# lauraflu/gr-doa

Measured on AMD Instinct MI355X. Metric: DoA snapshots/sec (autocorr+MUSIC+peak) @ N=4, 1024 samp, 1024 angles, higher is better.
Workload: dtype f32; 1 GPU; BASELINE.json configs[1]: 4-ch ULA, 1 source, K=1024 (overlap 0), P=1024, batch=4096 snapshots/step, complex fp32, SNR 20 dB; batch=4096, inputs=4, snapshot_size=1024, pspectrum_len=1024, num_targets=1, internal_precision=64, rotating_batches=8, hip_streams=4, parallelism=snapshot-sharded x1, no data-path collective

## Files before the change

### gr-doa_amd/csrc/autocorrelate.hip

```cpp
#include "common.hpp"

#include <cstdlib>

namespace doa {

struct CovArgs {
    const float2 *in[DOA_MAX_ANT_ELE];
    float2 *out;
    int n_ch;
    int K;
    int S;
    int n_out;
    int avg;
    float inv_k;
    float fb_hk;
    const float2 *gain;
    float2 *pieces;
    int q, r;
    int n_steps;
};

template <int TN> struct TriAcc {
    float d[TN];
    float re[TN * (TN - 1) / 2 > 0 ? TN * (TN - 1) / 2 : 1];
    float im[TN * (TN - 1) / 2 > 0 ? TN * (TN - 1) / 2 : 1];
};

template <int TN> __device__ __forceinline__ void tri_accumulate(TriAcc<TN> &acc, const float2 (&x)[TN])
{
    int idx = 0;
#pragma unroll
    for (int a = 0; a < TN; a++) {
        acc.d[a] = fmaf(x[a].x, x[a].x, fmaf(x[a].y, x[a].y, acc.d[a]));
#pragma unroll
        for (int b = a + 1; b < TN; b++) {
            acc.re[idx] = fmaf(x[a].x, x[b].x, fmaf(x[a].y, x[b].y, acc.re[idx]));
            acc.im[idx] = fmaf(x[a].y, x[b].x, fmaf(-x[a].x, x[b].y, acc.im[idx]));
            idx++;
        }
    }
}

template <int TN, bool VEC2, int UN, bool NT = false>
__global__ __launch_bounds__(256) void cov_wave_kernel(CovArgs g)
{
    const int lane = threadIdx.x & (kWave - 1);
    const int wave0 = blockIdx.x * (blockDim.x / kWave) + (threadIdx.x / kWave);
    const int n_waves = gridDim.x * (blockDim.x / kWave);
    for (int snap = wave0; snap < g.n_out; snap += n_waves) {
    const size_t base = (size_t)snap * (size_t)g.S;

    TriAcc<TN> acc;
#pragma unroll
    for (int a = 0; a < TN; a++) acc.d[a] = 0.f;
#pragma unroll
    for (int i = 0; i < TN * (TN - 1) / 2; i++) { acc.re[i] = 0.f; acc.im[i] = 0.f; }

    if constexpr (VEC2) {
        const int npair = g.K >> 1;
        int p = lane;
        for (; p + (UN - 1) * kWave < npair; p += UN * kWave) {
            float4 v[UN][TN];
#pragma unroll
            for (int u = 0; u < UN; u++)
#pragma unroll
                for (int a = 0; a < TN; a++)
                    v[u][a] = load_f4<NT>(reinterpret_cast<const float4 *>(g.in[a] + base + 2 * (size_t)(p + u * kWave)));
#pragma unroll
            for (int u = 0; u < UN; u++) {
                float2 x0[TN], x1[TN];
#pragma unroll
                for (int a = 0; a < TN; a++) { x0[a] = make_float2(v[u][a].x, v[u][a].y); x1[a] = make_float2(v[u][a].z, v[u][a].w); }
                tri_accumulate<TN>(acc, x0);
                tri_accumulate<TN>(acc, x1);
            }
        }
        for (; p < npair; p += kWave) {
            float4 v[TN];
#pragma unroll
            for (int a = 0; a < TN; a++) v[a] = load_f4<NT>(reinterpret_cast<const float4 *>(g.in[a] + base + 2 * (size_t)p));
            float2 x0[TN], x1[TN];
#pragma unroll
            for (int a = 0; a < TN; a++) { x0[a] = make_float2(v[a].x, v[a].y); x1[a] = make_float2(v[a].z, v[a].w); }
            tri_accumulate<TN>(acc, x0);
            tri_accumulate<TN>(acc, x1);
        }
        if ((g.K & 1) && lane == 0) {
            float2 x[TN];
#pragma unroll
            for (int a = 0; a < TN; a++) x[a] = g.in[a][base + (size_t)(g.K - 1)];
            tri_accumulate<TN>(acc, x);
        }
    } else {
#pragma unroll 4
        for (int t = lane; t < g.K; t += kWave) {
            float2 x[TN];
#pragma unroll
            for (int a = 0; a < TN; a++) x[a] = g.in[a][base + (size_t)t];
            tri_accumulate<TN>(acc, x);
        }
    }

#pragma unroll
    for (int a = 0; a < TN; a++) acc.d[a] = wave_allreduce_sum(acc.d[a]);
#pragma unroll
    for (int i = 0; i < TN * (TN - 1) / 2; i++) {
        acc.re[i] = wave_allreduce_sum(acc.re[i]);
        acc.im[i] = wave_allreduce_sum(acc.im[i]);
    }

    float2 r = make_float2(0.f, 0.f);
    {
        int idx = 0;
#pragma unroll
        for (int a = 0; a < TN; a++) {
            if (lane == a + a * TN) r = make_float2(acc.d[a], 0.f);
#pragma unroll
            for (int b = a + 1; b < TN; b++) {
                if (lane == a + b * TN) r = make_float2(acc.re[idx], acc.im[idx]);
                if (lane == b + a * TN) r = make_float2(acc.re[idx], -acc.im[idx]);
                idx++;
            }
        }
    }
    r.x = __fmul_rn(r.x, g.inv_k);
    r.y = __fmul_rn(r.y, g.inv_k);
    if (g.gain && lane < TN * TN) {
        const float2 w = g.gain[lane];
        r = make_float2(fmaf(w.x, r.x, -w.y * r.y), fmaf(w.x, r.y, w.y * r.x));
    }
    if (g.avg == 1) {
        const int src = (lane < TN * TN) ? (TN * TN - 1 - lane) : lane;
        const float px = __shfl(r.x, src, kWave);
        const float py = __shfl(r.y, src, kWave);
        r.x = __fadd_rn(__fmul_rn(0.5f, r.x), __fmul_rn(g.fb_hk, px));
        r.y = __fadd_rn(__fmul_rn(0.5f, r.y), __fmul_rn(g.fb_hk, -py));
    }
    if (lane < TN * TN) g.out[(size_t)snap * (TN * TN) + lane] = r;
    }
// ... 18 lines not shown
            for (int a = 0; a < TN; a++) { x0[a] = make_float2(v[u][a].x, v[u][a].y); x1[a] = make_float2(v[u][a].z, v[u][a].w); }
            tri_accumulate<TN>(acc, x0);
            tri_accumulate<TN>(acc, x1);
        }
    }
    for (; p < npair; p += kWave) {
        float4 v[TN];
#pragma unroll
        for (int a = 0; a < TN; a++) v[a] = load_f4<NT>(reinterpret_cast<const float4 *>(in[a] + first + 2 * (size_t)p));
        float2 x0[TN], x1[TN];
#pragma unroll
        for (int a = 0; a < TN; a++) { x0[a] = make_float2(v[a].x, v[a].y); x1[a] = make_float2(v[a].z, v[a].w); }
        tri_accumulate<TN>(acc, x0);
        tri_accumulate<TN>(acc, x1);
    }
}

template <int TN> __device__ __forceinline__ void tri_clear(TriAcc<TN> &acc)
{
#pragma unroll
    for (int a = 0; a < TN; a++) acc.d[a] = 0.f;
#pragma unroll
    for (int i = 0; i < TN * (TN - 1) / 2; i++) { acc.re[i] = 0.f; acc.im[i] = 0.f; }
}

template <int TN> __device__ __forceinline__ float2 tri_reduce_to_lane(TriAcc<TN> &acc, int lane)
{
#pragma unroll
    for (int a = 0; a < TN; a++) acc.d[a] = wave_allreduce_sum(acc.d[a]);
#pragma unroll
    for (int i = 0; i < TN * (TN - 1) / 2; i++) {
        acc.re[i] = wave_allreduce_sum(acc.re[i]);
        acc.im[i] = wave_allreduce_sum(acc.im[i]);
    }
    float2 r = make_float2(0.f, 0.f);
    int idx = 0;
#pragma unroll
    for (int a = 0; a < TN; a++) {
// ... 383 lines not shown
```

### gr-doa_amd/csrc/kernels.hpp

```cpp
#pragma once
#include "common.hpp"

namespace doa {

size_t autocorrelate_workspace_bytes(int N, int K, int ovl, int n_out);
int launch_autocorrelate(int N, int K, int ovl, int avg, int n_out, const void *const *d_in, void *d_out,
                         hipStream_t st, const void *d_gain_outer = nullptr, void *d_workspace = nullptr);

struct MusicTables {
    int N = 0, M = 0, P = 0;
    float norm_spacing = 0.f;
    DevBuf d_z;
    DevBuf d_zd;
    int build(float norm_spacing, int num_targets, int num_ant_ele, int pspectrum_len);
    void release() { d_z.release(); d_zd.release(); }
};

inline int coef_stride(int N) { return 2 * N; }

int launch_music_evd(int N, int M, int n_items, const void *d_R, void *d_coef, void *d_coef_d, void *d_pn,
                     int evd_bits, hipStream_t st, void *d_cheb = nullptr);
inline bool music_uses_cheb(int N, int bits) { return N <= 4 && bits == 64; }
constexpr int kChebRecord = 8;
long long evd_fallback_count(bool reset);
// ... 4 lines not shown
int launch_music_scan(const MusicTables &t, int bits, int n_items, const void *d_coef, void *d_spec, void *d_q,
                      hipStream_t st, const PeakTables *peaks = nullptr, void *d_max = nullptr,
                      void *d_argmax = nullptr, bool *peaks_done = nullptr, bool store_spectrum = true,
                      const void *d_cheb = nullptr);

struct PeakTables {
    int M = 0, L = 0;
    float x_min = 0.f, x_max = 0.f;
    DevBuf d_x;
    int build(int num_max_vals, int vector_len, float x_min, float x_max);
    void release() { d_x.release(); }
};
int launch_find_local_max(const PeakTables &t, int n_items, const void *d_in, void *d_max, void *d_argmax,
                          hipStream_t st);

int launch_root_music(int N, int M, float norm_spacing, int n_items, const void *d_coef, void *d_out,
                      void *d_status, hipStream_t st, void *d_roots = nullptr);
int launch_root_select(int N, int M, float norm_spacing, int n_items, const void *d_roots, void *d_out, void *d_status,
                       hipStream_t st);

}
```

### gr-doa_amd/csrc/music_evd.hip

```cpp
#include "jacobi.hpp"
#include "kernels.hpp"
#include <mutex>
#include <type_traits>

#include <cstdlib>

namespace doa {

}
#include "evd_subspace.hpp"
namespace doa {

__device__ __forceinline__ void write_cheb_record(double *__restrict__ o, const double (&ux)[4], const double (&uy)[4])
{
    o[0] = ux[0] - 2 * ux[2]; o[1] = 2 * ux[1] - 6 * ux[3]; o[2] = 4 * ux[2]; o[3] = 8 * ux[3];
    o[4] = 2 * uy[3] - 2 * uy[1]; o[5] = -4 * uy[2]; o[6] = -8 * uy[3]; o[7] = 0.0;
}

template <int N, typename T>
__global__ __launch_bounds__(64) void music_evd_kernel(const float2 *__restrict__ R, float *__restrict__ coef,
                                                       double *__restrict__ coef_d, float2 *__restrict__ pn_out,
                                                       int n_items, int M, double *__restrict__ cheb_d,
                                                       unsigned long long *__restrict__ fallback_count)
{
    const int item = blockIdx.x * blockDim.x + threadIdx.x;
    if (item >= n_items) return;
    T u[2 * N];
    const float2 *Ri = R + (size_t)item * (N * N);
    float2 *pn_i = pn_out ? pn_out + (size_t)item * (N * N) : nullptr;
    bool done = false;
    if constexpr (sizeof(T) == 8) {
        if (M == 1) {
            done = evd_small_subspace<N, 1>(Ri, u, pn_i);
            if (!done && fallback_count) atomicAdd(fallback_count, 1ull);
        }
    }
    if (!done) evd_item_coefficients<N, T>(Ri, M, u, pn_i);
    if (coef) {
#pragma unroll
        for (int k = 0; k < 2 * N; k++) coef[(size_t)item * (2 * N) + k] = (float)u[k];
    }
    if (coef_d) {
#pragma unroll
        for (int k = 0; k < 2 * N; k++) coef_d[(size_t)item * (2 * N) + k] = (double)u[k];
    }
    if (cheb_d) {
        const double ux[4] = {(double)u[0], (N > 1) ? (double)u[1] : 0.0, (N > 2) ? (double)u[3] : 0.0, (N > 3) ? (double)u[5] : 0.0};
        const double uy[4] = {0.0, (N > 1) ? (double)u[2] : 0.0, (N > 2) ? (double)u[4] : 0.0, (N > 3) ? (double)u[6] : 0.0};
        write_cheb_record(cheb_d + (size_t)item * kChebRecord, ux, uy);
    }
}

template <int G> struct Tournament {
    static constexpr int a(int t, int j) { return j == 0 ? G - 1 : (t + j) % (G - 1); }
    static constexpr int b(int t, int j) { return j == 0 ? t : (t - j + (G - 1)) % (G - 1); }
    static constexpr int p(int t, int j) { return a(t, j) < b(t, j) ? a(t, j) : b(t, j); }
    static constexpr int q(int t, int j) { return a(t, j) < b(t, j) ? b(t, j) : a(t, j); }
};

template <typename T> __device__ __forceinline__ T lane_fetch(T v, int src_lane);
template <> __device__ __forceinline__ float lane_fetch<float>(float v, int src_lane) { return __shfl(v, src_lane, kWave); }
template <> __device__ __forceinline__ double lane_fetch<double>(double v, int src_lane) { return __shfl(v, src_lane, kWave); }

template <int G, typename T> __device__ __forceinline__ T group_sum(T v, int lane)
{
// ... 967 lines not shown
```

### gr-doa_amd/csrc/pipeline.hip

```cpp
#include "kernels.hpp"
#include "pipeline_lanes.hpp"

#include <cstdlib>
#include <cstring>
#include <string>

namespace doa {
bool find_local_max_fast_ok(int L, const void *d_in);
int launch_find_local_max_serial(const PeakTables &t, int n_items, const void *d_in, void *d_max, void *d_argmax,
                                 void *d_scratch, hipStream_t st);
}

struct doa_music_pipeline {
    int N = 0, K = 0, ovl = 0, avg = 0;
    int max_batch = 0;
    int bits = 64;
    int device = 0;
    unsigned stages = 7;
    doa::MusicTables music;
    doa::PeakTables peaks;
    doa::DevBuf d_cov, d_coef, d_cheb, d_spec, d_scratch, d_gain;
    bool has_gain = false;
    hipStream_t hst[2] = {nullptr, nullptr};
    doa::DevBuf d_in[2], d_res;
    doa::DevBuf d_work[2];
    doa::PinnedBuf h_stage;
    int fail_chunk = -1;
    enum { kCoef = 0, kCheb, kCov, kSpec, kWork, kScratch };
    doa::PipeLanes lanes;
};

struct PipeWs {
    void *coef;
    void *cheb;
    void *spec_scratch;
    void *work;
    doa::DevBuf *scratch;
    size_t scratch_item_off;
};

static int run_k1(doa_music_pipeline *h, int n, const void *const *d_in, void *cov, const PipeWs &ws, hipStream_t st)
{
    if (~h->stages & 1u) return DOA_OK;
    return doa::launch_autocorrelate(h->N, h->K, h->ovl, h->avg, n, d_in, cov, st, h->has_gain ? h->d_gain.p : nullptr, ws.work);
// ... 33 lines not shown

static int run_dev(doa_music_pipeline *h, int n, const void *const *d_in, void *cov, void *spec, void *mx, void *am,
                   size_t item_off, hipStream_t st, int lane = 0)
{
    const bool dbl = (h->bits == 64);
    PipeWs ws;
    ws.coef = static_cast<char *>(h->d_coef.p) + item_off * doa::coef_stride(h->N) * (dbl ? sizeof(double) : sizeof(float));
    ws.cheb = h->d_cheb.p ? static_cast<char *>(h->d_cheb.p) + item_off * doa::kChebRecord * sizeof(double) : nullptr;
    ws.spec_scratch = static_cast<char *>(h->d_spec.p) + item_off * h->peaks.L * sizeof(float);
    ws.work = h->d_work[lane].p;
    ws.scratch = &h->d_scratch;
    ws.scratch_item_off = item_off;
    return run_ws(h, n, d_in, cov, spec, mx, am, ws, st);
}

extern "C" {

doa_music_pipeline_t *doa_music_pipeline_create(int inputs, int snapshot_size, int overlap_size, int avg_method,
                                                float norm_spacing, int num_targets, int pspectrum_len, int max_batch)
{
    doa::clear_error();
    if (inputs <= 0 || inputs > DOA_MAX_ANT_ELE || snapshot_size <= 0 || overlap_size < 0 ||
        overlap_size >= snapshot_size) {
        doa::set_error("music_pipeline: bad autocorrelate parameters (inputs=%d snapshot=%d overlap=%d)", inputs,
                       snapshot_size, overlap_size);
        return nullptr;
    }
    if (num_targets <= 0 || num_targets >= inputs || num_targets > DOA_MAX_PEAKS || !(norm_spacing > 0.0f) ||
        norm_spacing > 0.5f || pspectrum_len <= 0 || max_batch <= 0) {
        doa::set_error("music_pipeline: bad MUSIC parameters (norm_spacing=%g num_targets=%d inputs=%d "
// ... 17 lines not shown
    if (const size_t ws = doa::autocorrelate_workspace_bytes(inputs, snapshot_size, overlap_size, max_batch); ws && rc == DOA_OK)
        rc = h->d_work[0].reserve(ws);
    if (rc != DOA_OK) {
        doa_music_pipeline_destroy(h);
        return nullptr;
    }
    return h;
}

void doa_music_pipeline_destroy(doa_music_pipeline_t *h)
{
    if (!h) return;
    h->music.release();
    h->peaks.release();
    h->d_cov.release(); h->d_coef.release(); h->d_cheb.release(); h->d_spec.release(); h->d_scratch.release(); h->d_gain.release();
    h->d_res.release(); h->h_stage.release();
    for (auto &b : h->d_work) b.release();
    for (auto &b : h->d_in) b.release();
    for (auto st : h->hst)
        if (st) (void)hipStreamDestroy(st);
    h->lanes.release();
    delete h;
}

int doa_music_pipeline_fuse_antenna_correction(doa_music_pipeline_t *h, const float *gains_re_im)
{
    doa::clear_error();
    if (!h) return DOA_ERR_INVALID_ARG;
    if (!gains_re_im) { h->has_gain = false; return DOA_OK; }
    const int N = h->N;
    float2 w[DOA_MAX_ANT_ELE * DOA_MAX_ANT_ELE];
// ... 20 lines not shown
int doa_music_pipeline_work_dev(doa_music_pipeline_t *h, int noutput_items, const void *const *d_input_items,
                                void *d_cov_out, void *d_spectrum_out, void *d_max_out, void *d_argmax_out,
                                void *hip_stream)
{
    doa::clear_error();
    if (!h || noutput_items < 0 || !d_input_items || (noutput_items > 0 && (!d_max_out || !d_argmax_out))) {
        doa::set_error("music_pipeline_work_dev: bad arguments");
        return DOA_ERR_INVALID_ARG;
    }
    if (noutput_items > h->max_batch) {
        doa::set_error("music_pipeline_work_dev: noutput_items=%d exceeds max_batch=%d", noutput_items, h->max_batch);
        return DOA_ERR_INVALID_ARG;
    }
    if (noutput_items == 0) return 0;
    if (int brc = doa::bind_device(h->device); brc != DOA_OK) return brc;
    void *cov = d_cov_out ? d_cov_out : h->d_cov.p;
    void *spec = d_spectrum_out;
    return run_dev(h, noutput_items, d_input_items, cov, spec, d_max_out, d_argmax_out, 0,
                   static_cast<hipStream_t>(hip_stream));
}

int doa_music_pipeline_set_lanes(doa_music_pipeline_t *h, int n_lanes)
{
    doa::clear_error();
    if (!h || h->lanes.set_count(n_lanes) != DOA_OK) {
        doa::set_error("music_pipeline_set_lanes: need 1 <= n_lanes <= %d", doa::PipeLanes::kMaxLanes);
        return DOA_ERR_INVALID_ARG;
    }
    return DOA_OK;
}

int doa_music_pipeline_work_dev_batches(doa_music_pipeline_t *h, int n_batches, int noutput_items,
                                        const void *const *d_input_items, void *const *d_cov_out,
                                        void *const *d_spectrum_out, void *const *d_max_out, void *const *d_argmax_out,
// ... 6 lines not shown
    }
    if (noutput_items > h->max_batch) {
        doa::set_error("music_pipeline_work_dev_batches: noutput_items=%d exceeds max_batch=%d", noutput_items, h->max_batch);
        return DOA_ERR_INVALID_ARG;
    }
    for (int b = 0; b < n_batches; b++)
        if (noutput_items > 0 && (!d_max_out[b] || !d_argmax_out[b])) {
            doa::set_error("music_pipeline_work_dev_batches: batch %d has no peak output pointers", b);
            return DOA_ERR_INVALID_ARG;
        }
    if (n_batches == 0 || noutput_items == 0) return 0;
    if (int brc = doa::bind_device(h->device); brc != DOA_OK) return brc;
    const int N = h->N;
    const int fail_at = h->lanes.fail_batch;
    h->fail_chunk = -1;
    if (h->lanes.n_lanes == 1 && hip_stream != DOA_STREAM_DETACHED) {
        hipStream_t caller = static_cast<hipStream_t>(hip_stream);
        h->lanes.fail_batch = -1;
        for (int b = 0; b < n_batches; b++) {
            if (fail_at == b) {
                doa::set_error("music_pipeline_work_dev_batches: injected failure in batch %d", b);
                (void)hipStreamSynchronize(caller);
                return DOA_ERR_HIP;
            }
            void *cov = (d_cov_out && d_cov_out[b]) ? d_cov_out[b] : h->d_cov.p;
            const int rc = run_dev(h, noutput_items, d_input_items + (size_t)b * N, cov, d_spectrum_out ? d_spectrum_out[b] : nullptr,
                                   d_max_out[b], d_argmax_out[b], 0, caller);
            if (rc < 0) { (void)hipStreamSynchronize(caller); return rc; }
        }
        return n_batches * noutput_items;
// ... 200 lines not shown
```

### gr-doa_amd/csrc/pipeline_lanes.hpp

```cpp
#pragma once
#include "common.hpp"

#include <string>

namespace doa {

int create_lane_streams(const hipStream_t *have, int n_have, hipStream_t *out, int n_new);

inline int ensure_stream_pair(hipStream_t (&st)[2])
{
    for (int i = 0; i < 2; i++) {
        if (st[i]) continue;
        if (const int rc = create_lane_streams(&st[1 - i], st[1 - i] ? 1 : 0, &st[i], 1); rc != DOA_OK) return rc;
    }
    return DOA_OK;
}

struct PipeLane {
    hipStream_t st = nullptr;
    bool own_stream = true;
    hipEvent_t done = nullptr;
    static constexpr int kBufs = 6;
    DevBuf buf[kBufs];
};

struct PipeLanes {
    static constexpr int kMaxLanes = 8;
    PipeLane lanes[kMaxLanes];
    int n_lanes = 4;
    int next_lane = 0;
    hipEvent_t fork_ev = nullptr;
    int fail_batch = -1;

    void release()
    {
        for (auto &l : lanes) {
            for (auto &b : l.buf) b.release();
// ... 25 lines not shown
        return DOA_OK;
    }
    int synchronize()
    {
        for (auto &l : lanes)
            if (l.st) DOA_HIP_TRY(hipStreamSynchronize(l.st));
        return DOA_OK;
    }
    bool idle() const
    {
        for (auto &l : lanes)
            if (l.st && hipStreamQuery(l.st) != hipSuccess) return false;
        return true;
    }

    template <class Prepare, class Launch>
    int run_batches(const char *what, int n_batches, void *hip_stream, Prepare prepare, Launch launch)
    {
        const bool detached = (hip_stream == DOA_STREAM_DETACHED);
        hipStream_t caller = detached ? nullptr : static_cast<hipStream_t>(hip_stream);
        const int fail_at = fail_batch;
        fail_batch = -1;
        const int L = n_lanes;
        if (!detached && !fork_ev) DOA_HIP_TRY(hipEventCreateWithFlags(&fork_ev, hipEventDisableTiming));
        {
            hipStream_t have[kMaxLanes], fresh[kMaxLanes];
            int n_have = 0, n_new = 0;
            for (int l = 0; l < L; l++)
                if (lanes[l].st) have[n_have++] = lanes[l].st;
            if (n_have < L) {
                if (const int rc = create_lane_streams(have, n_have, fresh, L - n_have); rc != DOA_OK) return rc;
                for (int l = 0; l < L; l++)
                    if (!lanes[l].st) { lanes[l].st = fresh[n_new++]; lanes[l].own_stream = true; }
            }
        }
        for (int l = 0; l < L; l++) {
            auto &ln = lanes[l];
            if (!detached && !ln.done) DOA_HIP_TRY(hipEventCreateWithFlags(&ln.done, hipEventDisableTiming));
            if (const int rc = prepare(ln); rc != DOA_OK) return rc;
        }
        const int lane0 = next_lane % L;
        next_lane = (lane0 + n_batches) % L;
        const int used = n_batches < L ? n_batches : L;
        int rc = DOA_OK;
        auto fail = [&](hipError_t e, const char *step) {
            if (e != hipSuccess && rc >= 0) { set_error("%s: %s failed: %s", what, step, hipGetErrorString(e)); rc = DOA_ERR_HIP; }
        };
        if (!detached) {
            fail(hipEventRecord(fork_ev, caller), "fork record");
            for (int u = 0; u < used && rc >= 0; u++) fail(hipStreamWaitEvent(lanes[(lane0 + u) % L].st, fork_ev, 0), "fork wait");
// ... 26 lines not shown
```

### gr-doa_amd/python/doa/_lib.py

```python
from __future__ import annotations

import ctypes as C
import os

_HERE = os.path.dirname(os.path.abspath(__file__))
LIB_PATH = os.environ.get(
    "DOA_HIP_LIB", os.path.normpath(os.path.join(_HERE, "..", "..", "lib", "libdoa_hip.so")))


class DoaError(RuntimeError):

    def __init__(self, status: int, message: str):
        super().__init__(f"libdoa_hip: {message} (status {status})")
        self.status = status


if not os.path.exists(LIB_PATH):
    raise ImportError(
        f"{LIB_PATH} not found: build the HIP extension first (make -C gr-doa_amd, or "
        f"python -c 'import __graft_entry__ as g; g.build()'). There is no CPU fallback.")



def _preload_torch_hip_runtime() -> None:
# ... 63 lines not shown
    "doa_calibrate_lin_array_create": (_vp, [C.c_float, C.c_int, C.c_float]),
    "doa_calibrate_lin_array_destroy": (None, [_vp]),
    "doa_calibrate_lin_array_work": (C.c_int, [_vp, C.c_int, _vp, _vp]),
    "doa_calibrate_lin_array_work_dev": (C.c_int, [_vp, C.c_int, _vp, _vp, _vp]),
    "doa_music_pipeline_create": (_vp, [C.c_int, C.c_int, C.c_int, C.c_int, C.c_float, C.c_int, C.c_int, C.c_int]),
    "doa_music_pipeline_destroy": (None, [_vp]),
    "doa_music_pipeline_set_stages": (C.c_int, [_vp, C.c_int]),
    "doa_music_pipeline_work_dev": (C.c_int, [_vp, C.c_int, _vpp, _vp, _vp, _vp, _vp, _vp]),
    "doa_music_pipeline_work": (C.c_int, [_vp, C.c_int, _vpp, _vp, _vp, _vp, _vp]),
    "doa_music_pipeline_work_dev_batches": (C.c_int, [_vp, C.c_int, C.c_int, _vpp, _vpp, _vpp, _vpp, _vpp, _vp]),
    "doa_music_pipeline_set_lanes": (C.c_int, [_vp, C.c_int]),
    "doa_music_pipeline_set_lane_streams": (C.c_int, [_vp, C.c_int, _vpp]),
    "doa_music_pipeline_synchronize": (C.c_int, [_vp]),
    "doa_music_pipeline_inject_failure": (C.c_int, [_vp, C.c_int]),
    "doa_music_pipeline_lanes_idle": (C.c_int, [_vp]),
    "doa_compass_mean_create": (_vp, [C.c_int]),
    "doa_compass_mean_destroy": (None, [_vp]),
    "doa_compass_mean_work": (C.c_int, [_vp, C.c_int, _vp, _vp]),
    "doa_compass_mean_work_dev": (C.c_int, [_vp, C.c_int, _vp, _vp, _vp]),
    "doa_sim_source_create": (_vp, [C.c_int, C.c_int, C.c_float, _vp, _vp, _vp, _vp, C.c_float, C.c_ulonglong]),
    "doa_sim_source_destroy": (None, [_vp]),
    "doa_sim_source_seek": (C.c_int, [_vp, C.c_longlong]),
    "doa_sim_source_tell": (C.c_longlong, [_vp]),
    "doa_sim_source_work": (C.c_int, [_vp, C.c_int, _vpp]),
    "doa_sim_source_work_dev": (C.c_int, [_vp, C.c_int, _vpp, _vp]),
    "doa_root_pipeline_create": (_vp, [C.c_int, C.c_int, C.c_int, C.c_int, C.c_float, C.c_int, C.c_int]),
    "doa_root_pipeline_destroy": (None, [_vp]),
    "doa_root_pipeline_fuse_antenna_correction": (C.c_int, [_vp, _vp]),
    "doa_root_pipeline_work_dev": (C.c_int, [_vp, C.c_int, _vpp, _vp, _vp, _vp, _vp]),
    "doa_root_pipeline_work_dev_batches": (C.c_int, [_vp, C.c_int, C.c_int, _vpp, _vpp, _vpp, _vpp, _vp]),
# ... 41 lines not shown
```

### gr-doa_amd/python/doa/blocks.py

```python
from __future__ import annotations

import ctypes as C

import numpy as np

from . import _lib
from ._lib import lib, check, check_handle, ptr_array

_C64 = np.complex64
_F32 = np.float32


def _vp(a: np.ndarray) -> C.c_void_p:
    return C.c_void_p(a.ctypes.data)


DETACHED = "detached"


def _stream_ptr(stream) -> C.c_void_p:
    if stream is None:
        return C.c_void_p(0)
    if isinstance(stream, str) and stream == DETACHED:
        return C.c_void_p(2 ** 64 - 1)
# ... 317 lines not shown
            k = min(self.max_batch, n - done)
            am = output_items[0][done:done + k]
            mx = output_items[1][done:done + k] if len(output_items) > 1 else np.empty((k, self.num_targets), _F32)
            sp = output_items[2][done:done + k] if len(output_items) > 2 else None
            done += self.work(k, [a[done * S:] for a in input_items], mx, am, spectrum_out=sp)
        return done, self.forecast(done)

    def fuse_antenna_correction(self, correction) -> None:
        _fuse(lib.doa_music_pipeline_fuse_antenna_correction, self._h, correction, self.inputs)

    def set_stages(self, cov=True, evd=True, scan=True) -> None:
        check(lib.doa_music_pipeline_set_stages(self._h, (1 if cov else 0) | (2 if evd else 0) | (4 if scan else 0)))

    def inject_failure(self, chunk_index: int) -> None:
        check(lib.doa_music_pipeline_inject_failure(self._h, int(chunk_index)))

    def lanes_idle(self) -> bool:
        return bool(check(lib.doa_music_pipeline_lanes_idle(self._h)))

    def work_dev(self, noutput_items, d_input_ptrs, d_cov_ptr, d_spec_ptr, d_max_ptr, d_argmax_ptr, stream=None) -> int:
        return check(lib.doa_music_pipeline_work_dev(
            self._h, int(noutput_items), ptr_array(d_input_ptrs), C.c_void_p(int(d_cov_ptr or 0)),
            C.c_void_p(int(d_spec_ptr or 0)), C.c_void_p(int(d_max_ptr)), C.c_void_p(int(d_argmax_ptr)),
            _stream_ptr(stream)))

    def set_lanes(self, n_lanes: int) -> None:
        check(lib.doa_music_pipeline_set_lanes(self._h, int(n_lanes)))

    def set_lane_streams(self, streams) -> None:
        self._lane_streams = list(streams)
# ... 215 lines not shown
```

Measured before the change: 164.1 million snapshots/s.

## Add warp-specialized fused covariance+EVD+scan kernel for MUSIC pipeline

```diff
diff --git a/gr-doa_amd/csrc/autocorrelate.hip b/gr-doa_amd/csrc/autocorrelate.hip
--- a/gr-doa_amd/csrc/autocorrelate.hip
+++ b/gr-doa_amd/csrc/autocorrelate.hip
@@ -1,4 +1,4 @@
-#include "common.hpp"
+#include "cov_wave.hpp"
 
 #include <cstdlib>
 
@@ -20,27 +20,6 @@
     int n_steps;
 };
 
-template <int TN> struct TriAcc {
-    float d[TN];
-    float re[TN * (TN - 1) / 2 > 0 ? TN * (TN - 1) / 2 : 1];
-    float im[TN * (TN - 1) / 2 > 0 ? TN * (TN - 1) / 2 : 1];
-};
-
-template <int TN> __device__ __forceinline__ void tri_accumulate(TriAcc<TN> &acc, const float2 (&x)[TN])
-{
-    int idx = 0;
-#pragma unroll
-    for (int a = 0; a < TN; a++) {
-        acc.d[a] = fmaf(x[a].x, x[a].x, fmaf(x[a].y, x[a].y, acc.d[a]));
-#pragma unroll
-        for (int b = a + 1; b < TN; b++) {
-            acc.re[idx] = fmaf(x[a].x, x[b].x, fmaf(x[a].y, x[b].y, acc.re[idx]));
-            acc.im[idx] = fmaf(x[a].y, x[b].x, fmaf(-x[a].x, x[b].y, acc.im[idx]));
-            idx++;
-        }
-    }
-}
-
 template <int TN, bool VEC2, int UN, bool NT = false>
 __global__ __launch_bounds__(256) void cov_wave_kernel(CovArgs g)
 {
@@ -50,79 +29,7 @@
     for (int snap = wave0; snap < g.n_out; snap += n_waves) {
     const size_t base = (size_t)snap * (size_t)g.S;
 
-    TriAcc<TN> acc;
-#pragma unroll
-    for (int a = 0; a < TN; a++) acc.d[a] = 0.f;
-#pragma unroll
-    for (int i = 0; i < TN * (TN - 1) / 2; i++) { acc.re[i] = 0.f; acc.im[i] = 0.f; }
-
-    if constexpr (VEC2) {
-        const int npair = g.K >> 1;
-        int p = lane;
-        for (; p + (UN - 1) * kWave < npair; p += UN * kWave) {
-            float4 v[UN][TN];
-#pragma unroll
-            for (int u = 0; u < UN; u++)
-#pragma unroll
-                for (int a = 0; a < TN; a++)
-                    v[u][a] = load_f4<NT>(reinterpret_cast<const float4 *>(g.in[a] + base + 2 * (size_t)(p + u * kWave)));
-#pragma unroll
-            for (int u = 0; u < UN; u++) {
-                float2 x0[TN], x1[TN];
-#pragma unroll
-                for (int a = 0; a < TN; a++) { x0[a] = make_float2(v[u][a].x, v[u][a].y); x1[a] = make_float2(v[u][a].z, v[u][a].w); }
-                tri_accumulate<TN>(acc, x0);
-                tri_accumulate<TN>(acc, x1);
-            }
-        }
-        for (; p < npair; p += kWave) {
-            float4 v[TN];
-#pragma unroll
-            for (int a = 0; a < TN; a++) v[a] = load_f4<NT>(reinterpret_cast<const float4 *>(g.in[a] + base + 2 * (size_t)p));
-            float2 x0[TN], x1[TN];
-#pragma unroll
-            for (int a = 0; a < TN; a++) { x0[a] = make_float2(v[a].x, v[a].y); x1[a] = make_float2(v[a].z, v[a].w); }
-            tri_accumulate<TN>(acc, x0);
-            tri_accumulate<TN>(acc, x1);
-        }
-        if ((g.K & 1) && lane == 0) {
-            float2 x[TN];
-#pragma unroll
-            for (int a = 0; a < TN; a++) x[a] = g.in[a][base + (size_t)(g.K - 1)];
-            tri_accumulate<TN>(acc, x);
-        }
-    } else {
-#pragma unroll 4
-        for (int t = lane; t < g.K; t += kWave) {
-            float2 x[TN];
-#pragma unroll
-            for (int a = 0; a < TN; a++) x[a] = g.in[a][base + (size_t)t];
-            tri_accumulate<TN>(acc, x);
-        }
-    }
-
-#pragma unroll
-    for (int a = 0; a < TN; a++) acc.d[a] = wave_allreduce_sum(acc.d[a]);
-#pragma unroll
-    for (int i = 0; i < TN * (TN - 1) / 2; i++) {
-        acc.re[i] = wave_allreduce_sum(acc.re[i]);
-        acc.im[i] = wave_allreduce_sum(acc.im[i]);
-    }
-
-    float2 r = make_float2(0.f, 0.f);
-    {
-        int idx = 0;
-#pragma unroll
-        for (int a = 0; a < TN; a++) {
-            if (lane == a + a * TN) r = make_float2(acc.d[a], 0.f);
-#pragma unroll
-            for (int b = a + 1; b < TN; b++) {
-                if (lane == a + b * TN) r = make_float2(acc.re[idx], acc.im[idx]);
-                if (lane == b + a * TN) r = make_float2(acc.re[idx], -acc.im[idx]);
-                idx++;
-            }
-        }
-    }
+    float2 r = cov_wave_snapshot<TN, VEC2, UN, NT>(g.in, base, g.K, lane);
     r.x = __fmul_rn(r.x, g.inv_k);
     r.y = __fmul_rn(r.y, g.inv_k);
     if (g.gain && lane < TN * TN) {
@@ -171,14 +78,6 @@
         tri_accumulate<TN>(acc, x0);
         tri_accumulate<TN>(acc, x1);
     }
-}
-
-template <int TN> __device__ __forceinline__ void tri_clear(TriAcc<TN> &acc)
-{
-#pragma unroll
-    for (int a = 0; a < TN; a++) acc.d[a] = 0.f;
-#pragma unroll
-    for (int i = 0; i < TN * (TN - 1) / 2; i++) { acc.re[i] = 0.f; acc.im[i] = 0.f; }
 }
 
 template <int TN> __device__ __forceinline__ float2 tri_reduce_to_lane(TriAcc<TN> &acc, int lane)
diff --git a/gr-doa_amd/csrc/cov_wave.hpp b/gr-doa_amd/csrc/cov_wave.hpp
--- /dev/null
+++ b/gr-doa_amd/csrc/cov_wave.hpp
@@ -0,0 +1,118 @@
+#pragma once
+#include "common.hpp"
+
+namespace doa {
+
+template <int TN> struct TriAcc {
+    float d[TN];
+    float re[TN * (TN - 1) / 2 > 0 ? TN * (TN - 1) / 2 : 1];
+    float im[TN * (TN - 1) / 2 > 0 ? TN * (TN - 1) / 2 : 1];
+};
+
+template <int TN> __device__ __forceinline__ void tri_accumulate(TriAcc<TN> &acc, const float2 (&x)[TN])
+{
+    int idx = 0;
+#pragma unroll
+    for (int a = 0; a < TN; a++) {
+        acc.d[a] = fmaf(x[a].x, x[a].x, fmaf(x[a].y, x[a].y, acc.d[a]));
+#pragma unroll
+        for (int b = a + 1; b < TN; b++) {
+            acc.re[idx] = fmaf(x[a].x, x[b].x, fmaf(x[a].y, x[b].y, acc.re[idx]));
+            acc.im[idx] = fmaf(x[a].y, x[b].x, fmaf(-x[a].x, x[b].y, acc.im[idx]));
+            idx++;
+        }
+    }
+}
+
+template <int TN> __device__ __forceinline__ void tri_clear(TriAcc<TN> &acc)
+{
+#pragma unroll
+    for (int a = 0; a < TN; a++) acc.d[a] = 0.f;
+#pragma unroll
+    for (int i = 0; i < TN * (TN - 1) / 2; i++) { acc.re[i] = 0.f; acc.im[i] = 0.f; }
+}
+template <int TN, int UN, bool NT>
+__device__ __forceinline__ void cov_trip_issue(float4 (&v)[UN][TN], const float2 *const *in, size_t base, int p)
+{
+#pragma unroll
+    for (int u = 0; u < UN; u++)
+#pragma unroll
+        for (int a = 0; a < TN; a++)
+            v[u][a] = load_f4<NT>(reinterpret_cast<const float4 *>(in[a] + base + 2 * (size_t)(p + u * kWave)));
+}
+template <int TN, int UN> __device__ __forceinline__ void cov_trip_accumulate(TriAcc<TN> &acc, const float4 (&v)[UN][TN])
+{
+#pragma unroll
+    for (int u = 0; u < UN; u++) {
+        float2 x0[TN], x1[TN];
+#pragma unroll
+        for (int a = 0; a < TN; a++) { x0[a] = make_float2(v[u][a].x, v[u][a].y); x1[a] = make_float2(v[u][a].z, v[u][a].w); }
+        tri_accumulate<TN>(acc, x0);
+        tri_accumulate<TN>(acc, x1);
+    }
+}
+template <int TN, int UN, bool NT>
+__device__ __forceinline__ void cov_wave_rest(TriAcc<TN> &acc, const float2 *const *in, size_t base, int K, int p, int lane)
+{
+    const int npair = K >> 1;
+    for (; p + (UN - 1) * kWave < npair; p += UN * kWave) {
+        float4 v[UN][TN];
+        cov_trip_issue<TN, UN, NT>(v, in, base, p);
+        cov_trip_accumulate<TN, UN>(acc, v);
+    }
+    for (; p < npair; p += kWave) {
+        float4 v[1][TN];
+        cov_trip_issue<TN, 1, NT>(v, in, base, p);
+        cov_trip_accumulate<TN, 1>(acc, v);
+    }
+    if ((K & 1) && lane == 0) {
+        float2 x[TN];
+#pragma unroll
+        for (int a = 0; a < TN; a++) x[a] = in[a][base + (size_t)(K - 1)];
+        tri_accumulate<TN>(acc, x);
+    }
+}
+template <int TN> __device__ __forceinline__ float2 cov_wave_pick(TriAcc<TN> &acc, int lane)
+{
+#pragma unroll
+    for (int a = 0; a < TN; a++) acc.d[a] = wave_allreduce_sum(acc.d[a]);
+#pragma unroll
+    for (int i = 0; i < TN * (TN - 1) / 2; i++) {
+        acc.re[i] = wave_allreduce_sum(acc.re[i]);
+        acc.im[i] = wave_allreduce_sum(acc.im[i]);
+    }
+    float2 r = make_float2(0.f, 0.f);
+    int idx = 0;
+#pragma unroll
+    for (int a = 0; a < TN; a++) {
+        if (lane == a + a * TN) r = make_float2(acc.d[a], 0.f);
+#pragma unroll
+        for (int b = a + 1; b < TN; b++) {
+            if (lane == a + b * TN) r = make_float2(acc.re[idx], acc.im[idx]);
+            if (lane == b + a * TN) r = make_float2(acc.re[idx], -acc.im[idx]);
+            idx++;
+        }
+    }
+    return r;
+}
+
+template <int TN, bool VEC2, int UN, bool NT>
+__device__ __forceinline__ float2 cov_wave_snapshot(const float2 *const *in, size_t base, int K, int lane)
+{
+    TriAcc<TN> acc;
+    tri_clear<TN>(acc);
+    if constexpr (VEC2) {
+        cov_wave_rest<TN, UN, NT>(acc, in, base, K, lane, lane);
+    } else {
+#pragma unroll 4
+        for (int t = lane; t < K; t += kWave) {
+            float2 x[TN];
+#pragma unroll
+            for (int a = 0; a < TN; a++) x[a] = in[a][base + (size_t)t];
+            tri_accumulate<TN>(acc, x);
+        }
+    }
+    return cov_wave_pick<TN>(acc, lane);
+}
+
+}
diff --git a/gr-doa_amd/csrc/fused_step.hip b/gr-doa_amd/csrc/fused_step.hip
--- /dev/null
+++ b/gr-doa_amd/csrc/fused_step.hip
@@ -0,0 +1,188 @@
+#include "cov_wave.hpp"
+#include "music_evd_item.hpp"
+#include "music_scan_impl.hpp"
+
+namespace doa {
+
+namespace {
+
+constexpr int kLoaders = 4;
+constexpr int kScanners = 3;
+constexpr int kTurn = 4;
+constexpr int kFusedThreads = (kLoaders + 1 + kScanners) * kWave;
+constexpr int kFusedBlocksPerCu = 1;
+constexpr int kLoadUnroll = 8;
+
+struct FusedArgs {
+    const double *ztab;
+    const float *xaxis;
+    float *scratch;
+    unsigned long long *fallback;
+    int n;
+    int n_items;
+    int K;
+    float inv_k;
+    FusedBatch b[kFusedMaxBatches];
+};
+
+__device__ __forceinline__ void turn_barrier()
+{
+    asm volatile("" ::: "memory");
+    __builtin_amdgcn_s_waitcnt(0xc07f);
+    __builtin_amdgcn_s_barrier();
+    asm volatile("" ::: "memory");
+}
+
+template <int N, int CH>
+__global__ __launch_bounds__(kFusedThreads) __attribute__((amdgpu_waves_per_eu(2, 2))) void fused_step_kernel(FusedArgs g)
+{
+    constexpr int P = 256 * CH;
+    constexpr int RL = LeanRecord<N, double>::kLen;
+    __shared__ double zt[2 * P];
+    __shared__ float xs[P];
+    __shared__ float2 ring[2][kTurn][N * N];
+    __shared__ double rec[2][kTurn][RL];
+    for (int i = threadIdx.x; i < 2 * P; i += kFusedThreads) zt[i] = g.ztab[i];
+    for (int i = threadIdx.x; i < P; i += kFusedThreads) xs[i] = g.xaxis[i];
+    __syncthreads();
+
+    const int lane = threadIdx.x & (kWave - 1);
+    const int wave = __builtin_amdgcn_readfirstlane(threadIdx.x / kWave);
+    const int n_turns = (g.n_items + kTurn - 1) / kTurn;
+    const int my_turns = ((int)blockIdx.x < n_turns) ? (n_turns - (int)blockIdx.x + (int)gridDim.x - 1) / (int)gridDim.x : 0;
+    auto first_item = [&](int t) { return ((int)blockIdx.x + t * (int)gridDim.x) * kTurn; };
+    const int n_iter = my_turns + 2;
+    if (wave < kLoaders) {
+        constexpr int UN = kLoadUnroll;
+        const bool pre = (g.K >> 1) >= UN * kWave;
+        float4 pf[UN][N];
+        auto batch_of = [&](int item, int &j) -> const FusedBatch & { const int b = item / g.n; j = item - b * g.n; return g.b[b]; };
+        if (pre && my_turns > 0 && first_item(0) + wave < g.n_items) {
+            int j;
+            const FusedBatch &B = batch_of(first_item(0) + wave, j);
+            cov_trip_issue<N, UN, true>(pf, B.in, (size_t)j * (size_t)g.K, lane);
+        }
+        for (int t = 0; t < n_iter; t++) {
+            if (t < my_turns) {
+                for (int i = wave; i < kTurn; i += kLoaders) {
+                    const int item = first_item(t) + i;
+                    if (item >= g.n_items) break;
+                    int j;
+                    const FusedBatch &B = batch_of(item, j);
+                    const size_t base = (size_t)j * (size_t)g.K;
+                    TriAcc<N> acc;
+                    tri_clear<N>(acc);
+                    if (pre && i == wave) {
+                        cov_trip_accumulate<N, UN>(acc, pf);
+                        cov_wave_rest<N, 2, true>(acc, B.in, base, g.K, lane + UN * kWave, lane);
+                    } else {
+                        cov_wave_rest<N, 2, true>(acc, B.in, base, g.K, lane, lane);
+                    }
+                    float2 r = cov_wave_pick<N>(acc, lane);
+                    r.x = __fmul_rn(r.x, g.inv_k);
+                    r.y = __fmul_rn(r.y, g.inv_k);
+                    if (lane < N * N) {
+                        ring[t & 1][i][lane] = r;
+                        if (B.cov) B.cov[(size_t)j * (N * N) + lane] = r;
+                    }
+                }
+                if (pre && t + 1 < my_turns && first_item(t + 1) + wave < g.n_items) {
+                    int j;
+                    const FusedBatch &B = batch_of(first_item(t + 1) + wave, j);
+                    cov_trip_issue<N, UN, true>(pf, B.in, (size_t)j * (size_t)g.K, lane);
+                }
+            }
+            turn_barrier();
+        }
+    } else {
+        const int w = wave - kLoaders - 1;
+        for (int t = 0; t < n_iter; t++) {
+            if (wave == kLoaders) {
+                if (t >= 1 && t <= my_turns && lane < kTurn && first_item(t - 1) + lane < g.n_items) {
+                    double u[2 * N];
+                    music_evd_item<N, double>(ring[(t - 1) & 1][lane], 1, u, nullptr, g.fallback);
+                    write_cheb_record_from<N, double>(rec[(t - 1) & 1][lane], u);
+                }
+            }
+            if (w >= 0 && t >= 2) {
+                for (int i = w; i < kTurn; i += kScanners) {
+                    const int item = first_item(t - 2) + i;
+                    if (item >= g.n_items) break;
+                    const int b = item / g.n, j = item - b * g.n;
+                    const FusedBatch &B = g.b[b];
+                    double c[RL];
+#pragma unroll
+                    for (int k = 0; k < RL; k++) {
+                        const double v = rec[t & 1][i][k];
+                        const int lo = __builtin_amdgcn_readfirstlane(__double2loint(v));
+                        const int hi = __builtin_amdgcn_readfirstlane(__double2hiint(v));
+                        c[k] = __hiloint2double(hi, lo);
+                    }
+                    double zr[CH][4], zi[CH][4];
+                    lean_load_table<CH, double>(zt, lane, zr, zi);
+                    float *mx = B.mx + j, *am = B.am + j;
+                    if (B.spec)
+                        lean_scan_item<N, CH, double, false, true, true>(c, zr, zi, g.ztab, B.spec + (size_t)j * P, xs, mx, am, 1, lane);
+                    else
+                        lean_scan_item<N, CH, double, false, true, false>(c, zr, zi, g.ztab,
+                                                                          g.scratch + ((size_t)blockIdx.x * kScanners + w) * P, xs,
+                                                                          mx, am, 1, lane);
+                }
+            }
+            turn_barrier();
+        }
+    }
+}
+
+template <int N, int CH> void launch_fused_nc(const FusedArgs &g, int grid, hipStream_t st)
+{
+    hipLaunchKernelGGL((fused_step_kernel<N, CH>), dim3(grid), dim3(kFusedThreads), 0, st, g);
+}
+
+template <int N> void launch_fused_n(int P, const FusedArgs &g, int grid, hipStream_t st)
+{
+    if (P == 256) launch_fused_nc<N, 1>(g, grid, st);
+    else if (P == 512) launch_fused_nc<N, 2>(g, grid, st);
+    else launch_fused_nc<N, 4>(g, grid, st);
+}
+
+}
+
+bool fused_step_shape_ok(int N, int K, int P) { return N >= 2 && N <= 4 && K > 0 && K % 2 == 0 && (P == 256 || P == 512 || P == 1024); }
+
+size_t fused_step_scratch_bytes(int P) { return (size_t)cu_count() * kFusedBlocksPerCu * kScanners * P * sizeof(float); }
+
+int launch_fused_step(int N, int K, int P, int n, int n_batches, const FusedBatch *batches, const void *d_ztab,
+                      const void *d_xaxis, void *d_scratch, hipStream_t st)
+{
+    if (!fused_step_shape_ok(N, K, P) || n <= 0 || n_batches < 0) { set_error("fused step: unsupported shape"); return DOA_ERR_UNSUPPORTED; }
+    FusedArgs g;
+    memset(&g, 0, sizeof g);
+    g.ztab = static_cast<const double *>(d_ztab);
+    g.xaxis = static_cast<const float *>(d_xaxis);
+    g.scratch = static_cast<float *>(d_scratch);
+    g.fallback = evd_fallback_counter();
+    g.n = n;
+    g.K = K;
+    g.inv_k = (float)(1.0 / K);
+    int per_launch = (int)((INT_MAX - 2 * kTurn) / n);
+    if (per_launch > kFusedMaxBatches) per_launch = kFusedMaxBatches;
+    if (per_launch < 1) { set_error("fused step: %d items per batch is too many", n); return DOA_ERR_UNSUPPORTED; }
+    const int max_grid = cu_count() * kFusedBlocksPerCu;
+    for (int b0 = 0; b0 < n_batches; b0 += per_launch) {
+        const int nb = (n_batches - b0 < per_launch) ? n_batches - b0 : per_launch;
+        memcpy(g.b, batches + b0, sizeof(FusedBatch) * nb);
+        g.n_items = nb * n;
+        const int n_turns = (g.n_items + kTurn - 1) / kTurn;
+        const int grid = n_turns < max_grid ? n_turns : max_grid;
+        switch (N) {
+        case 2: launch_fused_n<2>(P, g, grid, st); break;
+        case 3: launch_fused_n<3>(P, g, grid, st); break;
+        default: launch_fused_n<4>(P, g, grid, st); break;
+        }
+        DOA_HIP_TRY(hipGetLastError());
+    }
+    return DOA_OK;
+}
+
+}
diff --git a/gr-doa_amd/csrc/kernels.hpp b/gr-doa_amd/csrc/kernels.hpp
--- a/gr-doa_amd/csrc/kernels.hpp
+++ b/gr-doa_amd/csrc/kernels.hpp
@@ -42,6 +42,18 @@
 int launch_find_local_max(const PeakTables &t, int n_items, const void *d_in, void *d_max, void *d_argmax,
                           hipStream_t st);
 
+struct FusedBatch {
+    const float2 *in[4];
+    float2 *cov;
+    float *spec;
+    float *mx, *am;
+};
+constexpr int kFusedMaxBatches = 56;
+bool fused_step_shape_ok(int N, int K, int P);
+size_t fused_step_scratch_bytes(int P);
+int launch_fused_step(int N, int K, int P, int n, int n_batches, const FusedBatch *batches, const void *d_ztab,
+                      const void *d_xaxis, void *d_scratch, hipStream_t st);
+
 int launch_root_music(int N, int M, float norm_spacing, int n_items, const void *d_coef, void *d_out,
                       void *d_status, hipStream_t st, void *d_roots = nullptr);
 int launch_root_select(int N, int M, float norm_spacing, int n_items, const void *d_roots, void *d_out, void *d_status,
diff --git a/gr-doa_amd/csrc/music_evd.hip b/gr-doa_amd/csrc/music_evd.hip
--- a/gr-doa_amd/csrc/music_evd.hip
+++ b/gr-doa_amd/csrc/music_evd.hip
@@ -1,21 +1,10 @@
-#include "jacobi.hpp"
-#include "kernels.hpp"
+#include "music_evd_item.hpp"
 #include <mutex>
 #include <type_traits>
 
 #include <cstdlib>
 
 namespace doa {
-
-}
-#include "evd_subspace.hpp"
-namespace doa {
-
-__device__ __forceinline__ void write_cheb_record(double *__restrict__ o, const double (&ux)[4], const double (&uy)[4])
-{
-    o[0] = ux[0] - 2 * ux[2]; o[1] = 2 * ux[1] - 6 * ux[3]; o[2] = 4 * ux[2]; o[3] = 8 * ux[3];
-    o[4] = 2 * uy[3] - 2 * uy[1]; o[5] = -4 * uy[2]; o[6] = -8 * uy[3]; o[7] = 0.0;
-}
 
 template <int N, typename T>
 __global__ __launch_bounds__(64) void music_evd_kernel(const float2 *__restrict__ R, float *__restrict__ coef,
@@ -28,14 +17,7 @@
     T u[2 * N];
     const float2 *Ri = R + (size_t)item * (N * N);
     float2 *pn_i = pn_out ? pn_out + (size_t)item * (N * N) : nullptr;
-    bool done = false;
-    if constexpr (sizeof(T) == 8) {
-        if (M == 1) {
-            done = evd_small_subspace<N, 1>(Ri, u, pn_i);
-            if (!done && fallback_count) atomicAdd(fallback_count, 1ull);
-        }
-    }
-    if (!done) evd_item_coefficients<N, T>(Ri, M, u, pn_i);
+    music_evd_item<N, T>(Ri, M, u, pn_i, fallback_count);
     if (coef) {
 #pragma unroll
         for (int k = 0; k < 2 * N; k++) coef[(size_t)item * (2 * N) + k] = (float)u[k];
@@ -44,11 +26,7 @@
 #pragma unroll
         for (int k = 0; k < 2 * N; k++) coef_d[(size_t)item * (2 * N) + k] = (double)u[k];
     }
-    if (cheb_d) {
-        const double ux[4] = {(double)u[0], (N > 1) ? (double)u[1] : 0.0, (N > 2) ? (double)u[3] : 0.0, (N > 3) ? (double)u[5] : 0.0};
-        const double uy[4] = {0.0, (N > 1) ? (double)u[2] : 0.0, (N > 2) ? (double)u[4] : 0.0, (N > 3) ? (double)u[6] : 0.0};
-        write_cheb_record(cheb_d + (size_t)item * kChebRecord, ux, uy);
-    }
+    if (cheb_d) write_cheb_record_from<N, T>(cheb_d + (size_t)item * kChebRecord, u);
 }
 
 template <int G> struct Tournament {
diff --git a/gr-doa_amd/csrc/music_evd_item.hpp b/gr-doa_amd/csrc/music_evd_item.hpp
--- /dev/null
+++ b/gr-doa_amd/csrc/music_evd_item.hpp
@@ -0,0 +1,35 @@
+#pragma once
+#include "jacobi.hpp"
+#include "kernels.hpp"
+#include "evd_subspace.hpp"
+
+namespace doa {
+
+__device__ __forceinline__ void write_cheb_record(double *__restrict__ o, const double (&ux)[4], const double (&uy)[4])
+{
+    o[0] = ux[0] - 2 * ux[2]; o[1] = 2 * ux[1] - 6 * ux[3]; o[2] = 4 * ux[2]; o[3] = 8 * ux[3];
+    o[4] = 2 * uy[3] - 2 * uy[1]; o[5] = -4 * uy[2]; o[6] = -8 * uy[3]; o[7] = 0.0;
+}
+
+template <int N, typename T> __device__ __forceinline__ void write_cheb_record_from(double *__restrict__ o, const T (&u)[2 * N])
+{
+    const double ux[4] = {(double)u[0], (N > 1) ? (double)u[1] : 0.0, (N > 2) ? (double)u[3] : 0.0, (N > 3) ? (double)u[5] : 0.0};
+    const double uy[4] = {0.0, (N > 1) ? (double)u[2] : 0.0, (N > 2) ? (double)u[4] : 0.0, (N > 3) ? (double)u[6] : 0.0};
+    write_cheb_record(o, ux, uy);
+}
+
+template <int N, typename T>
+__device__ __forceinline__ void music_evd_item(const float2 *__restrict__ Ri, int M, T (&u)[2 * N], float2 *__restrict__ pn_i,
+                                              unsigned long long *__restrict__ fallback_count)
+{
+    bool done = false;
+    if constexpr (sizeof(T) == 8) {
+        if (M == 1) {
+            done = evd_small_subspace<N, 1>(Ri, u, pn_i);
+            if (!done && fallback_count) atomicAdd(fallback_count, 1ull);
+        }
+    }
+    if (!done) evd_item_coefficients<N, T>(Ri, M, u, pn_i);
+}
+
+}
diff --git a/gr-doa_amd/csrc/pipeline.hip b/gr-doa_amd/csrc/pipeline.hip
--- a/gr-doa_amd/csrc/pipeline.hip
+++ b/gr-doa_amd/csrc/pipeline.hip
@@ -4,6 +4,7 @@
 #include <cstdlib>
 #include <cstring>
 #include <string>
+#include <vector>
 
 namespace doa {
 bool find_local_max_fast_ok(int L, const void *d_in);
@@ -26,8 +27,11 @@
     doa::DevBuf d_work[2];
     doa::PinnedBuf h_stage;
     int fail_chunk = -1;
-    enum { kCoef = 0, kCheb, kCov, kSpec, kWork, kScratch };
+    enum { kCoef = 0, kCheb, kCov, kSpec, kWork, kScratch, kFusedRows };
     doa::PipeLanes lanes;
+    int fused_mode = 1;
+    int fused_calls = 0;
+    doa::DevBuf d_fused_rows;
 };
 
 struct PipeWs {
@@ -91,6 +95,40 @@
     return run_ws(h, n, d_in, cov, spec, mx, am, ws, st);
 }
 
+static bool fused_eligible(const doa_music_pipeline *h, bool serial, int n_batches, const void *const *d_in, void *const *cov,
+                           void *const *spec)
+{
+    if (h->fused_mode == 0 || (h->fused_mode == 1 && !serial) || h->stages != 7u || h->bits != 64 || h->has_gain || h->ovl != 0 || h->avg != 0 || h->music.M != 1 ||
+        h->peaks.L != h->music.P || !doa::fused_step_shape_ok(h->N, h->K, h->music.P))
+        return false;
+    for (int b = 0; b < n_batches; b++) {
+        for (int k = 0; k < h->N; k++) {
+            const void *p = d_in[(size_t)b * h->N + k];
+            if (!p || reinterpret_cast<uintptr_t>(p) % 16) return false;
+        }
+        if (cov && cov[b] && reinterpret_cast<uintptr_t>(cov[b]) % 8) return false;
+        if (spec && spec[b] && reinterpret_cast<uintptr_t>(spec[b]) % 16) return false;
+    }
+    return true;
+}
+
+static int run_fused(doa_music_pipeline *h, int n_batches, int n, const void *const *d_in, void *const *cov, void *const *spec,
+                     void *const *mx, void *const *am, doa::DevBuf &rows, hipStream_t st)
+{
+    int rc = rows.reserve(doa::fused_step_scratch_bytes(h->music.P));
+    if (rc != DOA_OK || n_batches == 0) return rc;
+    std::vector<doa::FusedBatch> tab((size_t)n_batches);
+    for (int b = 0; b < n_batches; b++) {
+        doa::FusedBatch &e = tab[b];
+        for (int k = 0; k < 4; k++) e.in[k] = k < h->N ? static_cast<const float2 *>(d_in[(size_t)b * h->N + k]) : nullptr;
+        e.cov = cov ? static_cast<float2 *>(cov[b]) : nullptr;
+        e.spec = spec ? static_cast<float *>(spec[b]) : nullptr;
+        e.mx = static_cast<float *>(mx[b]);
+        e.am = static_cast<float *>(am[b]);
+    }
+    return doa::launch_fused_step(h->N, h->K, h->music.P, n, n_batches, tab.data(), h->music.d_zd.p, h->peaks.d_x.p, rows.p, st);
+}
+
 extern "C" {
 
 doa_music_pipeline_t *doa_music_pipeline_create(int inputs, int snapshot_size, int overlap_size, int avg_method,
@@ -138,7 +176,7 @@
     h->music.release();
     h->peaks.release();
     h->d_cov.release(); h->d_coef.release(); h->d_cheb.release(); h->d_spec.release(); h->d_scratch.release(); h->d_gain.release();
-    h->d_res.release(); h->h_stage.release();
+    h->d_res.release(); h->h_stage.release(); h->d_fused_rows.release();
     for (auto &b : h->d_work) b.release();
     for (auto &b : h->d_in) b.release();
     for (auto st : h->hst)
@@ -189,10 +227,32 @@
     }
     if (noutput_items == 0) return 0;
     if (int brc = doa::bind_device(h->device); brc != DOA_OK) return brc;
+    if (fused_eligible(h, true, 1, d_input_items, &d_cov_out, &d_spectrum_out)) {
+        const int rc = run_fused(h, 1, noutput_items, d_input_items, &d_cov_out, &d_spectrum_out, &d_max_out, &d_argmax_out,
+                                 h->d_fused_rows, static_cast<hipStream_t>(hip_stream));
+        if (rc != DOA_OK) return rc;
+        h->fused_calls++;
+        return noutput_items;
+    }
     void *cov = d_cov_out ? d_cov_out : h->d_cov.p;
     void *spec = d_spectrum_out;
     return run_dev(h, noutput_items, d_input_items, cov, spec, d_max_out, d_argmax_out, 0,
                    static_cast<hipStream_t>(hip_stream));
+}
+
+int doa_music_pipeline_set_fused_step(doa_music_pipeline_t *h, int mode)
+{
+    doa::clear_error();
+    if (!h || mode < 0 || mode > 2) { doa::set_error("music_pipeline_set_fused_step: bad arguments"); return DOA_ERR_INVALID_ARG; }
+    h->fused_mode = mode;
+    return DOA_OK;
+}
+
+int doa_music_pipeline_fused_calls_debug(doa_music_pipeline_t *h)
+{
+    doa::clear_error();
+    if (!h) { doa::set_error("music_pipeline_fused_calls_debug: bad arguments"); return DOA_ERR_INVALID_ARG; }
+    return h->fused_calls;
 }
 
 int doa_music_pipeline_set_lanes(doa_music_pipeline_t *h, int n_lanes)
@@ -229,6 +289,35 @@
     const int N = h->N;
     const int fail_at = h->lanes.fail_batch;
     h->fail_chunk = -1;
+    if (fused_eligible(h, h->lanes.n_lanes == 1, n_batches, d_input_items, d_cov_out, d_spectrum_out)) {
+        const bool attached = (hip_stream != DOA_STREAM_DETACHED);
+        h->lanes.fail_batch = -1;
+        hipStream_t st = static_cast<hipStream_t>(hip_stream);
+        doa::DevBuf *rows = &h->d_fused_rows;
+        if (h->lanes.n_lanes > 1 || !attached) {
+            if (const int rc = h->lanes.ensure_streams(); rc != DOA_OK) return rc;
+            const int L = h->lanes.n_lanes, lane0 = h->lanes.next_lane % L;
+            h->lanes.next_lane = (lane0 + n_batches) % L;
+            if (!attached) {
+                st = h->lanes.lanes[lane0].st;
+                rows = &h->lanes.lanes[lane0].buf[doa_music_pipeline::kFusedRows];
+            }
+        }
+        const int nb = (fail_at >= 0 && fail_at < n_batches) ? fail_at : n_batches;
+        int rc = run_fused(h, nb, noutput_items, d_input_items, d_cov_out, d_spectrum_out, d_max_out, d_argmax_out, *rows, st);
+        if (rc == DOA_OK && nb < n_batches) {
+            doa::set_error("music_pipeline_work_dev_batches: injected failure in batch %d", nb);
+            rc = DOA_ERR_HIP;
+        }
+        if (rc != DOA_OK) {
+            const std::string msg = doa_last_error();
+            (void)hipStreamSynchronize(st);
+            doa::set_error("%s", msg.c_str());
+            return rc;
+        }
+        h->fused_calls++;
+        return n_batches * noutput_items;
+    }
     if (h->lanes.n_lanes == 1 && hip_stream != DOA_STREAM_DETACHED) {
         hipStream_t caller = static_cast<hipStream_t>(hip_stream);
         h->lanes.fail_batch = -1;
diff --git a/gr-doa_amd/csrc/pipeline_lanes.hpp b/gr-doa_amd/csrc/pipeline_lanes.hpp
--- a/gr-doa_amd/csrc/pipeline_lanes.hpp
+++ b/gr-doa_amd/csrc/pipeline_lanes.hpp
@@ -20,7 +20,7 @@
     hipStream_t st = nullptr;
     bool own_stream = true;
     hipEvent_t done = nullptr;
-    static constexpr int kBufs = 6;
+    static constexpr int kBufs = 7;
     DevBuf buf[kBufs];
 };
 
@@ -76,6 +76,21 @@
         return true;
     }
 
+    int ensure_streams()
+    {
+        const int L = n_lanes;
+        hipStream_t have[kMaxLanes], fresh[kMaxLanes];
+        int n_have = 0, n_new = 0;
+        for (int l = 0; l < L; l++)
+            if (lanes[l].st) have[n_have++] = lanes[l].st;
+        if (n_have < L) {
+            if (const int rc = create_lane_streams(have, n_have, fresh, L - n_have); rc != DOA_OK) return rc;
+            for (int l = 0; l < L; l++)
+                if (!lanes[l].st) { lanes[l].st = fresh[n_new++]; lanes[l].own_stream = true; }
+        }
+        return DOA_OK;
+    }
+
     template <class Prepare, class Launch>
     int run_batches(const char *what, int n_batches, void *hip_stream, Prepare prepare, Launch launch)
     {
@@ -85,17 +100,7 @@
         fail_batch = -1;
         const int L = n_lanes;
         if (!detached && !fork_ev) DOA_HIP_TRY(hipEventCreateWithFlags(&fork_ev, hipEventDisableTiming));
-        {
-            hipStream_t have[kMaxLanes], fresh[kMaxLanes];
-            int n_have = 0, n_new = 0;
-            for (int l = 0; l < L; l++)
-                if (lanes[l].st) have[n_have++] = lanes[l].st;
-            if (n_have < L) {
-                if (const int rc = create_lane_streams(have, n_have, fresh, L - n_have); rc != DOA_OK) return rc;
-                for (int l = 0; l < L; l++)
-                    if (!lanes[l].st) { lanes[l].st = fresh[n_new++]; lanes[l].own_stream = true; }
-            }
-        }
+        if (const int rc = ensure_streams(); rc != DOA_OK) return rc;
         for (int l = 0; l < L; l++) {
             auto &ln = lanes[l];
             if (!detached && !ln.done) DOA_HIP_TRY(hipEventCreateWithFlags(&ln.done, hipEventDisableTiming));
diff --git a/gr-doa_amd/python/doa/_lib.py b/gr-doa_amd/python/doa/_lib.py
--- a/gr-doa_amd/python/doa/_lib.py
+++ b/gr-doa_amd/python/doa/_lib.py
@@ -101,6 +101,8 @@
     "doa_music_pipeline_synchronize": (C.c_int, [_vp]),
     "doa_music_pipeline_inject_failure": (C.c_int, [_vp, C.c_int]),
     "doa_music_pipeline_lanes_idle": (C.c_int, [_vp]),
+    "doa_music_pipeline_set_fused_step": (C.c_int, [_vp, C.c_int]),
+    "doa_music_pipeline_fused_calls_debug": (C.c_int, [_vp]),
     "doa_compass_mean_create": (_vp, [C.c_int]),
     "doa_compass_mean_destroy": (None, [_vp]),
     "doa_compass_mean_work": (C.c_int, [_vp, C.c_int, _vp, _vp]),
diff --git a/gr-doa_amd/python/doa/blocks.py b/gr-doa_amd/python/doa/blocks.py
--- a/gr-doa_amd/python/doa/blocks.py
+++ b/gr-doa_amd/python/doa/blocks.py
@@ -355,6 +355,12 @@
 
     def inject_failure(self, chunk_index: int) -> None:
         check(lib.doa_music_pipeline_inject_failure(self._h, int(chunk_index)))
+
+    def set_fused_step(self, mode: int = 1) -> None:
+        check(lib.doa_music_pipeline_set_fused_step(self._h, int(mode)))
+
+    def fused_calls(self) -> int:
+        return check(lib.doa_music_pipeline_fused_calls_debug(self._h))
 
     def lanes_idle(self) -> bool:
         return bool(check(lib.doa_music_pipeline_lanes_idle(self._h)))
```

Result: slower. 161.6 million snapshots/s (median of 2 runs) (-1.5%).
